# romanwerpachowski/ML

Hardware: NVIDIA B200
Metric: em_point_components_per_second (higher is better)
Workload: dtype f64

## Files before the change

### ml_b200/csrc/em.cu

```cuda
#include <algorithm>
#include <cmath>
#include <cstring>
#include <limits>

#include "em_direct.cuh"
#include "em_split.cuh"
#include "fastmath.cuh"
#include "internal.h"

namespace mlb {

constexpr int kTile = 64;
constexpr int kEmThreads = 128;
constexpr int kLogBatch = 16;

#ifdef MLB_EM_LIBM_EXP
#define MLB_EM_EXP(x) exp(x)
#else
#define MLB_EM_EXP(x) exp_nonpositive((x), etab)
#endif
#ifndef MLB_EM_MINB_SMALL
#define MLB_EM_MINB_SMALL 4
#endif

// ... 27 lines not shown
    int chunk;
    int n_chunks;
    unsigned* counter;
    const double* r_in;
    long long r_ld;
    double* r_out;
    long long r_out_ld;
    unsigned* labels_out;
    long long range_begin, range_count;
};

__device__ __forceinline__ long long min64(long long a, long long b) { return a < b ? a : b; }

__device__ __forceinline__ void dmma(double (&acc)[2], double a, double b)
{
    asm("mma.sync.aligned.m8n8k4.row.col.f64.f64.f64.f64 {%0,%1}, {%2}, {%3}, {%0,%1};" : "+d"(acc[0]), "+d"(acc[1]) : "d"(a), "d"(b));
}

template <int NT>
__device__ __forceinline__ void load_theta_frag(const double* thE, int j, int lane, double (&bf)[NT])
{
    if constexpr (NT == 1) {
        bf[0] = thE[j * 32 + lane];
    } else {
#pragma unroll
        for (int h = 0; h < NT / 2; ++h) {
            const double2 v = reinterpret_cast<const double2*>(thE)[(j * (NT / 2) + h) * 32 + lane];
            bf[2 * h] = v.x;
            bf[2 * h + 1] = v.y;
        }
    }
}

template <int DP, int KP, int MODE>
__global__ void __launch_bounds__(kEmThreads, (DP * KP <= 128 || MODE == 2) ? MLB_EM_MINB_SMALL : 2) em_kernel(const EmArgs p)
{
    constexpr int NT = KP / 8, DQ = DP / 4, NE = em_ne(DP), NM = em_nm(DP);
    constexpr int ZS = DP + 4, RS = KP + 4;
    constexpr int WN = (NM >= 8 || NT == 1) ? 1 : 2, WM = 4 / WN;
    constexpr int MW = (NM + WM - 1) / WM, NW = NT / WN;
    constexpr int SV = em_sv(DP, KP);
    constexpr int XR = kTile * DP / kEmThreads;

    extern __shared__ __align__(16) double sm[];
    double* thE = sm;
    double* cE = thE + NE * NT * 32;
    double* Zb = cE + KP;
    double* R = Zb + 2 * kTile * ZS;
    double* wl = R + kTile * RS;
    double* sh = wl + 8;
    double* etab = sh + DP;
    __shared__ int s_next;

    const int tid = threadIdx.x, lane = tid & 31, warp = tid >> 5, g = lane >> 2, c = lane & 3;
    const int d = p.d;

    if (MODE != 1)
        for (int i = tid; i < em_theta_len(DP, KP); i += kEmThreads) sm[i] = p.theta[i];
    for (int i = tid; i < 2 * kTile * ZS; i += kEmThreads) Zb[i] = 0.0;
    for (int i = tid; i < kTile * RS; i += kEmThreads) R[i] = 0.0;
    if (tid < DP) sh[tid] = tid < d ? p.shift[tid] : 0.0;
    load_exp_table(etab);

    const int wm = warp / WN, wn = warp % WN;
    int ia[MW], ib[MW];
    double sacc[MW][NW][2];
    if (MODE != 2) {
#pragma unroll
        for (int i = 0; i < MW; ++i) {
            const int mt = wm * MW + i;
            const int2 f = mt < NM ? p.feat_m[mt * 8 + g] : make_int2(DP + 1, DP + 1);
            ia[i] = f.x;
            ib[i] = f.y;
// ... 32 lines not shown
        if (tid == 0) s_next = static_cast<int>(atomicAdd(p.counter, 1u));
        __syncthreads();
        const int chunk = s_next;
        if (chunk >= p.n_chunks) break;
        const long long p_begin = work_begin + static_cast<long long>(chunk) * p.chunk;
        const long long p_end = min64(p_begin + p.chunk, work_end);
        const int ntiles = static_cast<int>((p_end - p_begin + kTile - 1) / kTile);

        if (MODE != 2) {
#pragma unroll
            for (int i = 0; i < MW; ++i)
#pragma unroll
                for (int nt = 0; nt < NW; ++nt) sacc[i][nt][0] = sacc[i][nt][1] = 0.0;
        }
        double ll_acc = 0.0, ll_prod = 1.0;

        load_tile(p_begin, static_cast<int>(min64(kTile, p_end - p_begin)));
        store_tile(Zb, static_cast<int>(min64(kTile, p_end - p_begin)));
        __syncthreads();

        for (int t = 0; t < ntiles; ++t) {
            double* Z = Zb + (t & 1) * kTile * ZS;
            const long long tile0 = p_begin + static_cast<long long>(t) * kTile;
            const int nvalid = static_cast<int>(min64(kTile, p_end - tile0));
            const int nvalid_next = t + 1 < ntiles ? static_cast<int>(min64(kTile, p_end - tile0 - kTile)) : 0;
            if (t + 1 < ntiles) load_tile(tile0 + kTile, nvalid_next);

            if (MODE == 1) {
                for (int idx = tid; idx < kTile * p.k; idx += kEmThreads) {
                    const int pt = idx % kTile, kk = idx / kTile;
                    R[pt * RS + kk] = pt < nvalid ? p.r_in[tile0 + pt + kk * p.r_ld] : 0.0;
                }
            } else {
                const double* z0 = Z + (warp * 16 + g) * ZS;
                const double* z1 = z0 + 8 * ZS;
                double acc[2][NT][2];
#pragma unroll
                for (int nt = 0; nt < NT; ++nt) {
                    const double2 cc = *reinterpret_cast<const double2*>(cE + 8 * nt + 2 * c);
                    acc[0][nt][0] = acc[1][nt][0] = cc.x;
                    acc[0][nt][1] = acc[1][nt][1] = cc.y;
                }
                double zc0[DQ], zc1[DQ];
#pragma unroll
                for (int m = 0; m < DQ; ++m) {
                    zc0[m] = z0[4 * m + c];
                    zc1[m] = z1[4 * m + c];
                }
                auto estep = [&](int j, double a0, double a1) {
                    double bf[NT];
                    load_theta_frag<NT>(thE, j, lane, bf);
#pragma unroll
                    for (int nt = 0; nt < NT; ++nt) {
                        dmma(acc[0][nt], a0, bf[nt]);
                        dmma(acc[1][nt], a1, bf[nt]);
                    }
                };
#pragma unroll
                for (int a = 0; a < DP - 4; ++a) {
                    const double za0 = z0[a], za1 = z1[a];
#pragma unroll
                    for (int m = a / 4 + 1; m < DQ; ++m) estep(em_estep_offdiag(DP, a, m), za0 * zc0[m], za1 * zc1[m]);
                }
                constexpr int J0 = em_ne_offdiag(DP);
#pragma unroll
                for (int m = 0; m < DQ; ++m) estep(J0 + m, zc0[m] * zc0[m], zc1[m] * zc1[m]);
#pragma unroll
                for (int m = 0; m < DQ; ++m) {
                    const int o = 4 * m + ((c + 1) & 3);
                    estep(J0 + DQ + m, zc0[m] * z0[o], zc1[m] * z1[o]);
                }
#pragma unroll
                for (int h = 0; h < (DQ + 1) / 2; ++h) {
                    const int mx = 2 * h + (c >> 1);
                    const int o = 4 * mx + c, o2 = 4 * mx + ((c + 2) & 3);
                    const bool live = mx < DQ;
                    const double u0 = live ? z0[o] * z0[o2] : 0.0, u1 = live ? z1[o] * z1[o2] : 0.0;
                    estep(J0 + 2 * DQ + h, u0, u1);
                }
#pragma unroll
                for (int m = 0; m < DQ; ++m) estep(NE - DQ + m, zc0[m], zc1[m]);
                double mxs[2], sums[2];
#pragma unroll
                for (int mt = 0; mt < 2; ++mt) {
#ifdef MLB_EM_FMAX_SHIFT
                    double mx = -INFINITY;
#pragma unroll
                    for (int nt = 0; nt < NT; ++nt) mx = fmax(mx, fmax(acc[mt][nt][0], acc[mt][nt][1]));
                    mx = fmax(mx, __shfl_xor_sync(0xffffffffu, mx, 1));
                    mx = fmax(mx, __shfl_xor_sync(0xffffffffu, mx, 2));
#else
                    int mkey = lse_key(acc[mt][0][0]);
#pragma unroll
                    for (int nt = 0; nt < NT; ++nt) mkey = max(mkey, max(lse_key(acc[mt][nt][0]), lse_key(acc[mt][nt][1])));
                    mkey = max(mkey, __shfl_xor_sync(0xffffffffu, mkey, 1));
                    mkey = max(mkey, __shfl_xor_sync(0xffffffffu, mkey, 2));
                    const double mx = lse_shift_of_key(mkey);
#endif
                    double sum = 0.0;
#pragma unroll
                    for (int nt = 0; nt < NT; ++nt) {
                        acc[mt][nt][0] = MLB_EM_EXP(acc[mt][nt][0] - mx);
                        acc[mt][nt][1] = MLB_EM_EXP(acc[mt][nt][1] - mx);
                        sum += acc[mt][nt][0] + acc[mt][nt][1];
                    }
                    sum += __shfl_xor_sync(0xffffffffu, sum, 1);
                    sum += __shfl_xor_sync(0xffffffffu, sum, 2);
                    mxs[mt] = mx;
                    sums[mt] = sum;
                }
                const double inv_mine = reciprocal_of_sum((c & 1) ? sums[1] : sums[0]);
                const double invs[2] = {__shfl_sync(0xffffffffu, inv_mine, lane & ~1), __shfl_sync(0xffffffffu, inv_mine, lane | 1)};
#pragma unroll
                for (int mt = 0; mt < 2; ++mt) {
                    const int pl = warp * 16 + mt * 8 + g;
                    const double inv = invs[mt];
                    if (c == 0 && pl < nvalid) {
                        ll_acc += mxs[mt];
                        ll_prod *= sums[mt];
                    }
                    if (MODE == 0) {
#pragma unroll
                        for (int nt = 0; nt < NT; ++nt)
                            *reinterpret_cast<double2*>(R + pl * RS + 8 * nt + 2 * c) = make_double2(acc[mt][nt][0] * inv, acc[mt][nt][1] * inv);
                    } else {
                        double best = -1.0;
                        unsigned best_k = 0xffffffffu;
#pragma unroll
                        for (int nt = 0; nt < NT; ++nt)
#pragma unroll
                            for (int e = 0; e < 2; ++e) {
                                const int kk = 8 * nt + 2 * c + e;
                                const double r = acc[mt][nt][e] * inv;
                                if (kk < p.k) {
                                    if (pl < nvalid && p.r_out) p.r_out[(tile0 - p.range_begin) + pl + kk * p.r_out_ld] = r;
                                    if (r > best) { best = r; best_k = kk; }
                                }
                            }
#pragma unroll
                        for (int off = 1; off <= 2; off <<= 1) {
                            const double ob = __shfl_xor_sync(0xffffffffu, best, off);
                            const unsigned ok = __shfl_xor_sync(0xffffffffu, best_k, off);
                            if (ob > best || (ob == best && ok < best_k)) { best = ob; best_k = ok; }
// ... 16 lines not shown
                        if (wm * MW + i < NM) {
                            const double af = zp[ia[i]] * zp[ib[i]];
#pragma unroll
                            for (int nt = 0; nt < NW; ++nt) dmma(sacc[i][nt], af, bf[nt]);
                        }
                    }
                }
            }
            if (MODE != 1 && ((t & (kLogBatch - 1)) == kLogBatch - 1 || t + 1 == ntiles)) {
                ll_acc += log(ll_prod);
                ll_prod = 1.0;
            }
            if (t + 1 < ntiles) store_tile(Zb + ((t + 1) & 1) * kTile * ZS, nvalid_next);
            __syncthreads();
        }

        if (MODE != 2) {
            double* out = p.partials + static_cast<long long>(chunk) * SV;
#pragma unroll
            for (int i = 0; i < MW; ++i) {
                const int mt = wm * MW + i;
                if (mt < NM) {
#pragma unroll
                    for (int nt = 0; nt < NW; ++nt)
                        *reinterpret_cast<double2*>(out + (mt * 8 + g) * KP + (wn * NW + nt) * 8 + 2 * c) = make_double2(sacc[i][nt][0], sacc[i][nt][1]);
                }
            }
#pragma unroll
            for (int off = 16; off >= 1; off >>= 1) ll_acc += __shfl_xor_sync(0xffffffffu, ll_acc, off);
            if (lane == 0) wl[warp] = ll_acc;
            __syncthreads();
            if (tid == 0) out[NM * 8 * KP] = (wl[0] + wl[1]) + (wl[2] + wl[3]);
            if (tid >= 1 && tid < 8) out[NM * 8 * KP + tid] = 0.0;
        }
    }
}

#include "em_small.cuh"

struct EmFinalizeArgs {
    const double* vsum;
    const double* dstats;
    const double* shift;
    int d, k, DP, KP, SV;
    int DPd, dSV;
    long long n_total;
    const int2* feat_m;
    const int2* feat_e;
    int nm8, ne;
    double* means;
    double* covs;
    double* weights;
    double* inv_covs;
    double* sqrt_dets;
    double* theta_out;
    double* dimg_out;
    double* kappa_out;
    int p_in_smem;
    double* ll_ring;
    unsigned long long* ll_counter;
    int ll_ring_len;
};

__global__ void em_finalize_kernel(const EmFinalizeArgs p)
{
    extern __shared__ double fs[];
// ... 161 lines not shown
    if (p.ll_ring && (p.vsum || p.dstats) && kc == 0 && tid == 0) {
        const double ll_sum = p.vsum ? tree8(p.vsum + (p.SV - 8), p.SV) : tree8(p.dstats + (p.dSV - 8), p.dSV);
        const unsigned long long idx = *p.ll_counter;
        p.ll_ring[idx % p.ll_ring_len] = ll_sum / static_cast<double>(p.n_total) - 0.5 * d * log(2.0 * 3.14159265358979323846);
        *p.ll_counter = idx + 1;
    }
}

__global__ void selftest_exp_kernel(const double* x, long long n, double* out)
{
    __shared__ double etab[kExpTableSize];
    load_exp_table(etab);
    __syncthreads();
    const long long i = static_cast<long long>(blockIdx.x) * blockDim.x + threadIdx.x;
    if (i < n) out[i] = exp_nonpositive(x[i], etab);
}


using EmKernelFn = void (*)(EmArgs);

template <int MODE>
static EmKernelFn em_kernel_for(int DP, int KP)
{
#define MLB_EM_CASE(D_, K_) if (DP == D_ && KP == K_) return em_kernel<D_, K_, MODE>;
#define MLB_EM_SMALL_CASE(D_, K_) if (DP == D_ && KP == K_) return em_small_kernel<D_, K_, MODE>;
    MLB_EM_SMALL_CASE(4, 8) MLB_EM_SMALL_CASE(4, 16) MLB_EM_SMALL_CASE(4, 32)
    MLB_EM_SMALL_CASE(8, 8) MLB_EM_SMALL_CASE(8, 16) MLB_EM_SMALL_CASE(8, 32)
    MLB_EM_CASE(16, 8) MLB_EM_CASE(16, 16) MLB_EM_CASE(16, 32)
#undef MLB_EM_CASE
#undef MLB_EM_SMALL_CASE
    return nullptr;
}

struct EmGpu {
    double* theta[2] = {nullptr, nullptr};
    double* params = nullptr;
    double* partials = nullptr;
    double* vsum = nullptr;
    double* ll = nullptr;
    unsigned long long* ll_counter = nullptr;
    int2* feat_m = nullptr;
    int2* feat_e = nullptr;
    unsigned* counter = nullptr;
    double* stage = nullptr;
    unsigned* stage_labels = nullptr;
    int grid = 0;
    double* r = nullptr;
    double* ll_tile = nullptr;
    int2* feat_e_off = nullptr;
    int grid_e = 0, grid_m = 0;
    KernelTimer timer;
};

using EmSplitKernelFn = void (*)(EmSplitArgs);

struct EmDirectGpu {
    double* img = nullptr;
    double* kappa = nullptr;
    double* r = nullptr;
    double* ll_tile = nullptr;
    double* partials = nullptr;
    double* vsum = nullptr;
    long long* sc_begin = nullptr;
    int2* tile_tab = nullptr;
    int n_sc = 0;
    int grid_e = 0, grid_m = 0;
};

struct EmDirect {
    bool capable = false;
    bool ready = false;
    int DP = 0, NB = 0, KPr = 0, IMG = 0, L = 0, SVd = 0;
    int cb = 1, cg = 1, tiles_per_range = 0, n_ranges = 1;
    size_t smem_e = 0, smem_m = 0;
    int64_t sc_bounds[kVirtualShards + 1] = {};
    std::vector<EmDirectGpu> gpus;
    ReduceScratch scratch;
};

constexpr int kDirectMaxDim = 128;
constexpr double kKappaDirect = 3.0e5;

constexpr int kLlRing = 4096;
constexpr long long kStagePoints = 1 << 20;

}

using namespace mlb;

struct mlb_em {
    mlb_ctx* ctx = nullptr;
    mlb_data* data = nullptr;
    int d = 0, k = 0, DP = 0, KP = 0, NT = 0, NE = 0, NM = 0, SV = 0;
    std::vector<int2> feat_m, feat_e;
    std::vector<EmGpu> gpus;
    int cur = 0;
    bool have_params = false, have_step = false;
    int last_path = 0;
    int64_t direct_steps = 0;
    int64_t launches = 0;
    int64_t steps_done = 0;
    EmKernelFn fn_step = nullptr, fn_mstep = nullptr, fn_emit = nullptr;
    int path = 1;
    EmDirect dr;
    int forced_path = 0;
    int route = 1;
    double kappa_max = 0.0;
    bool r_direct_valid = false;
    double* kappa_host = nullptr;
    EmSplitKernelFn fn_split_e = nullptr, fn_split_m = nullptr;
    size_t smem_split_e = 0, smem_split_m = 0;
    size_t smem_fused = 0;
    int MW = 4;
    cudaGraphExec_t step_graph[2] = {nullptr, nullptr};
    int64_t launches_per_step = 0;
    int plain_steps = 0;
    ReduceScratch reduce_scratch;

    double* means(int g) const { return gpus[g].params; }
    double* covs(int g) const { return gpus[g].params + d * k; }
    double* weights(int g) const { return covs(g) + static_cast<size_t>(k) * d * d; }
    double* inv_covs(int g) const { return weights(g) + k; }
    double* sqrt_dets(int g) const { return inv_covs(g) + static_cast<size_t>(k) * d * d; }
    size_t params_len() const { return static_cast<size_t>(d) * k + 2 * static_cast<size_t>(k) * d * d + 2 * k; }
};

namespace mlb {

static int pad_to(int v, const int* options, int n)
{
    for (int i = 0; i < n; ++i)
        if (v <= options[i]) return options[i];
    return 0;
}

static EmArgs base_args(const mlb_em* em, int g)
{
    const DataShard& sh = em->data->shards[g];
    const EmGpu& eg = em->gpus[g];
    EmArgs a{};
    a.x = sh.x;
    a.n_local = sh.n();
    a.d = em->d;
    a.k = em->k;
    a.shift = sh.shift;
    a.theta = eg.theta[em->cur];
    a.feat_m = eg.feat_m;
    a.partials = eg.partials;
    a.chunk = em->data->lay.chunk;
    a.n_chunks = static_cast<int>(sh.n_chunks());
    a.counter = eg.counter;
    return a;
}

static int launch_em(mlb_em* em, EmKernelFn fn, const EmArgs& a, int g, int grid)
{
    Gpu& gpu = em->ctx->gpus[g];
    MLB_CUDA(cudaMemsetAsync(a.counter, 0, sizeof(unsigned), gpu.stream));
    if (a.n_chunks > 0) {
        const bool timed = fn == em->fn_step;
        if (timed) MLB_TRY(em->gpus[g].timer.begin(gpu.stream));
        fn<<<std::min(grid, a.n_chunks), em->DP <= 8 ? kSmallThreads : kEmThreads, em->smem_fused, gpu.stream>>>(a);
        MLB_CUDA(cudaGetLastError());
        if (timed) MLB_TRY(em->gpus[g].timer.end(gpu.stream));
        ++em->launches;
    }
    return MLB_OK;
}

static EmSplitArgs split_args(const mlb_em* em, int g, const double* theta)
{
    const DataShard& sh = em->data->shards[g];
    const EmGpu& eg = em->gpus[g];
    EmSplitArgs a{};
    a.x = sh.x;
    a.n_local = sh.n();
    a.d = em->d; a.k = em->k; a.DP = em->DP; a.KP = em->KP;
    a.shift = sh.shift;
    a.theta = theta;
    a.feat_e = eg.feat_e_off;
    a.feat_m = eg.feat_m;
    a.ne = em->NE; a.nm = em->NM;
    a.r = eg.r;
    a.partials = eg.partials;
    a.ll_tile = eg.ll_tile;
    a.sv = em->SV;
    a.chunk = em->data->lay.chunk;
    a.n_chunks = static_cast<int>(sh.n_chunks());
    a.counter = eg.counter;
    return a;
}

static int launch_split(mlb_em* em, int g, const double* theta, bool run_e, bool timed)
{
    Gpu& gpu = em->ctx->gpus[g];
    EmGpu& eg = em->gpus[g];
    const EmSplitArgs a = split_args(em, g, theta);
    if (a.n_chunks == 0) return MLB_OK;
    if (timed) MLB_TRY(eg.timer.begin(gpu.stream));
    if (run_e) {
        MLB_CUDA(cudaMemsetAsync(a.counter, 0, sizeof(unsigned), gpu.stream));
        const long long e_items = static_cast<long long>(a.n_chunks) * (a.chunk / kSpTile);
        em->fn_split_e<<<static_cast<unsigned>(std::min<long long>(eg.grid_e, e_items)), kSpThreads, em->smem_split_e, gpu.stream>>>(a);
        MLB_CUDA(cudaGetLastError());
        ++em->launches;
    }
    const int ngroups = em->KP / (em->NT * 8), nslabs = (em->NM + 4 * em->MW - 1) / (4 * em->MW);
    const long long nitems = static_cast<long long>(a.n_chunks) * nslabs * ngroups;
    MLB_REQUIRE(nitems < (1ll << 31), "EM split path: too many work items");
    MLB_CUDA(cudaMemsetAsync(a.counter, 0, sizeof(unsigned), gpu.stream));
    em->fn_split_m<<<static_cast<unsigned>(std::min<long long>(eg.grid_m, nitems)), kSpThreads, em->smem_split_m, gpu.stream>>>(a);
    MLB_CUDA(cudaGetLastError());
    ++em->launches;
    if (timed) MLB_TRY(eg.timer.end(gpu.stream));
    return MLB_OK;
}

static int launch_pass(mlb_em* em, int g, const double* theta, bool timed)
{
    if (em->path == 2) return launch_split(em, g, theta, true, timed);
    EmArgs a = base_args(em, g);
    a.theta = theta;
    return launch_em(em, em->fn_step, a, g, em->gpus[g].grid);
}

static EmFinalizeArgs finalize_args(const mlb_em* em, int g, int stats, int theta_slot, bool want_ll)
{
    const EmGpu& eg = em->gpus[g];
    EmFinalizeArgs f{};
    f.vsum = stats == 1 ? eg.vsum : nullptr;
    f.shift = em->data->shards[g].shift;
    f.d = em->d; f.k = em->k; f.DP = em->DP; f.KP = em->KP; f.SV = em->SV;
    f.n_total = em->data->lay.n_total;
    f.feat_m = eg.feat_m; f.feat_e = eg.feat_e;
    f.nm8 = em->NM * 8; f.ne = em->NE;
    f.means = em->means(g); f.covs = em->covs(g); f.weights = em->weights(g);
    f.inv_covs = em->inv_covs(g); f.sqrt_dets = em->sqrt_dets(g);
    f.theta_out = em->path ? eg.theta[theta_slot] : nullptr;
    if (em->dr.capable) {
        const EmDirectGpu& dg = em->dr.gpus[g];
        f.DPd = em->dr.DP; f.dSV = em->dr.SVd;
        f.dstats = stats == 2 ? dg.vsum : nullptr;
        f.dimg_out = dg.img;
        f.kappa_out = dg.kappa;
    }
    f.ll_ring = want_ll ? eg.ll : nullptr;
    f.ll_counter = eg.ll_counter;
    f.ll_ring_len = kLlRing;
    return f;
}

static size_t finalize_smem(const mlb_em* em, bool* p_in_smem)
{
    const size_t d = static_cast<size_t>(em->d);
    const size_t with_p = sizeof(double) * (2 * d * d + 3 * d), without = sizeof(double) * (d * d + 3 * d);
    const bool fits = with_p <= 200 * 1024;
// ... 407 lines not shown
    MLB_CUDA(cudaMemcpy(out, dy, sizeof(double) * n, cudaMemcpyDeviceToHost));
    MLB_CUDA(cudaFree(dx));
    MLB_CUDA(cudaFree(dy));
    return MLB_OK;
}

int mlb_em_create(mlb_ctx* ctx, mlb_data* data, int k, mlb_em** out)
{
    MLB_ENTER(ctx);
    MLB_REQUIRE(ctx && data && out, "mlb_em_create: null argument");
    MLB_REQUIRE(data->ctx == ctx, "mlb_em_create: data belongs to another context");
    MLB_REQUIRE(k >= 1, "mlb_em_create: number of components must be positive");
    MLB_REQUIRE(data->d <= kDirectMaxDim, "mlb_em_create: D=%d not supported by this build (D <= %d)", data->d, kDirectMaxDim);
    static const int dps[] = {4, 8, 16}, kps[] = {8, 16, 32};
    const bool fused = data->d <= 16 && k <= 32;
    const bool split = !fused && data->d <= 64 && k <= 256;
    int DP = 0, KP = 0, NT = 0;
    if (fused) {
        DP = pad_to(data->d, dps, 3);
        KP = pad_to(k, kps, 3);
        NT = KP / 8;
    } else if (split) {
        DP = (data->d + 3) / 4 * 4;
        const int KG = k > 32 ? 64 : (k > 16 ? 32 : 16);
        KP = (k + KG - 1) / KG * KG;
        NT = KG / 8;
    }
    auto* em = new mlb_em;
    em->ctx = ctx; em->data = data; em->d = data->d; em->k = k;
    em->path = fused ? 1 : split ? 2 : 0;
    em->route = em->path ? em->path : 3;
    if (const char* env = std::getenv("MLB200_EM_PATH"))
        if (std::strcmp(env, "direct") == 0) em->forced_path = 3;
    if (em->path) {
        em->DP = DP; em->KP = KP; em->NT = NT; em->NE = em_ne(DP); em->NM = em_nm(DP); em->SV = em_sv(DP, KP);
    }
    if (fused) {
        em->fn_step = em_kernel_for<0>(DP, KP);
        em->fn_mstep = em_kernel_for<1>(DP, KP);
        em->fn_emit = em_kernel_for<2>(DP, KP);
        em->smem_fused = DP <= 8 ? em_small_smem_bytes(DP, KP) : em_smem_bytes(DP, KP);
    } else if (split) {
        em->fn_split_e = NT == 8 ? em_split_e_kernel<8> : NT == 4 ? em_split_e_kernel<4> : em_split_e_kernel<2>;
        int best_waste = 1 << 30;
        for (int mw = 3; mw <= 5; ++mw) {
            const int slabs = (em->NM + 4 * mw - 1) / (4 * mw), waste = slabs * 4 * mw - em->NM;
            if (waste <= best_waste) { best_waste = waste; em->MW = mw; }
        }
        if (NT == 8) em->fn_split_m = em->MW == 3 ? em_split_m_kernel<8, 3> : em->MW == 4 ? em_split_m_kernel<8, 4> : em_split_m_kernel<8, 5>;
        else if (NT == 4) em->fn_split_m = em->MW == 3 ? em_split_m_kernel<4, 3> : em->MW == 4 ? em_split_m_kernel<4, 4> : em_split_m_kernel<4, 5>;
        else em->fn_split_m = em->MW == 3 ? em_split_m_kernel<2, 3> : em->MW == 4 ? em_split_m_kernel<2, 4> : em_split_m_kernel<2, 5>;
        em->smem_split_e = em_split_e_smem(NT, DP, KP);
        em->smem_split_m = em_split_m_smem(NT, DP);
    }
    if (em->path) {
        em->feat_e.assign(static_cast<size_t>(em->NE) * 4, make_int2(-1, -1));
        const int DQ = DP / 4, J0 = em_ne_offdiag(DP);
        auto put = [&](int j, int c, int a, int b) { em->feat_e[static_cast<size_t>(j) * 4 + c] = make_int2(std::min(a, b), std::max(a, b)); };
        for (int a = 0; a < DP - 4; ++a)
            for (int m = a / 4 + 1; m < DQ; ++m)
                for (int c = 0; c < 4; ++c) put(em_estep_offdiag(DP, a, m), c, a, 4 * m + c);
        for (int m = 0; m < DQ; ++m)
            for (int c = 0; c < 4; ++c) {
                put(J0 + m, c, 4 * m + c, 4 * m + c);
                put(J0 + DQ + m, c, 4 * m + c, 4 * m + ((c + 1) & 3));
            }
        for (int h = 0; h < (DQ + 1) / 2; ++h)
            for (int c = 0; c < 4; ++c) {
                const int mx = 2 * h + (c >> 1);
                if (mx < DQ) put(J0 + 2 * DQ + h, c, 4 * mx + c, 4 * mx + ((c + 2) & 3));
            }
// ... 48 lines not shown
    int rc = for_each_gpu(ctx, [&](int g, Gpu& gpu) -> int {
        EmGpu& eg = em->gpus[g];
        EmDirectGpu& dg = em->dr.gpus[g];
        const DataShard& sh = data->shards[g];
        MLB_CUDA(cudaMallocFromPoolAsync(&eg.params, sizeof(double) * em->params_len(), gpu.pool, gpu.stream));
        MLB_CUDA(cudaMallocFromPoolAsync(&eg.ll, sizeof(double) * kLlRing, gpu.pool, gpu.stream));
        MLB_CUDA(cudaMallocFromPoolAsync(&eg.ll_counter, sizeof(unsigned long long), gpu.pool, gpu.stream));
        MLB_CUDA(cudaMemsetAsync(eg.ll_counter, 0, sizeof(unsigned long long), gpu.stream));
        MLB_CUDA(cudaMallocFromPoolAsync(&eg.counter, sizeof(unsigned), gpu.pool, gpu.stream));
        MLB_CUDA(cudaMallocFromPoolAsync(&dg.img, sizeof(double) * static_cast<size_t>(k) * em->dr.IMG, gpu.pool, gpu.stream));
        MLB_CUDA(cudaMallocFromPoolAsync(&dg.kappa, sizeof(double) * k, gpu.pool, gpu.stream));
        MLB_CUDA(cudaMemsetAsync(dg.kappa, 0, sizeof(double) * k, gpu.stream));
        {
            const size_t fin_smem = finalize_smem(em, nullptr);
            if (fin_smem > 48 * 1024)
                MLB_CUDA(cudaFuncSetAttribute(reinterpret_cast<const void*>(em_finalize_kernel), cudaFuncAttributeMaxDynamicSharedMemorySize, static_cast<int>(fin_smem)));
        }
        int sms = 0;
        MLB_CUDA(cudaDeviceGetAttribute(&sms, cudaDevAttrMultiProcessorCount, gpu.device));
        if (em->path) {
            const size_t theta_len = static_cast<size_t>(em_theta_len(DP, KP));
            MLB_CUDA(cudaMallocFromPoolAsync(&eg.theta[0], sizeof(double) * theta_len, gpu.pool, gpu.stream));
            MLB_CUDA(cudaMallocFromPoolAsync(&eg.theta[1], sizeof(double) * theta_len, gpu.pool, gpu.stream));
            MLB_CUDA(cudaMallocFromPoolAsync(&eg.partials, sizeof(double) * std::max<int64_t>(1, sh.n_chunks()) * em->SV, gpu.pool, gpu.stream));
            MLB_CUDA(cudaMallocFromPoolAsync(&eg.vsum, sizeof(double) * kVirtualShards * em->SV, gpu.pool, gpu.stream));
            MLB_CUDA(cudaMallocFromPoolAsync(&eg.feat_m, sizeof(int2) * em->feat_m.size(), gpu.pool, gpu.stream));
            MLB_CUDA(cudaMallocFromPoolAsync(&eg.feat_e, sizeof(int2) * em->feat_e.size(), gpu.pool, gpu.stream));
            MLB_CUDA(cudaMemsetAsync(eg.vsum, 0, sizeof(double) * kVirtualShards * em->SV, gpu.stream));
            MLB_CUDA(cudaMemcpyAsync(eg.feat_m, em->feat_m.data(), sizeof(int2) * em->feat_m.size(), cudaMemcpyHostToDevice, gpu.stream));
            MLB_CUDA(cudaMemcpyAsync(eg.feat_e, em->feat_e.data(), sizeof(int2) * em->feat_e.size(), cudaMemcpyHostToDevice, gpu.stream));
        }
        if (em->path == 1) {
            const size_t smem = em->smem_fused;
            for (EmKernelFn fn : {em->fn_step, em->fn_mstep, em->fn_emit})
                MLB_CUDA(cudaFuncSetAttribute(reinterpret_cast<const void*>(fn), cudaFuncAttributeMaxDynamicSharedMemorySize, static_cast<int>(smem)));
            int per_sm = 0;
            MLB_CUDA(cudaOccupancyMaxActiveBlocksPerMultiprocessor(&per_sm, reinterpret_cast<const void*>(em->fn_step), em->DP <= 8 ? kSmallThreads : kEmThreads, smem));
            MLB_REQUIRE(per_sm >= 1, "mlb_em_create: EM kernel does not fit on an SM");
            eg.grid = per_sm * sms;
        } else if (em->path == 2) {
            std::vector<int2> off(em->feat_e.size());
            for (size_t i = 0; i < off.size(); ++i) off[i] = em->feat_e[i].x < 0 ? make_int2(DP + 1, DP + 1) : em->feat_e[i];
            MLB_CUDA(cudaMallocFromPoolAsync(&eg.feat_e_off, sizeof(int2) * off.size(), gpu.pool, gpu.stream));
            MLB_CUDA(cudaMemcpyAsync(eg.feat_e_off, off.data(), sizeof(int2) * off.size(), cudaMemcpyHostToDevice, gpu.stream));
            MLB_CUDA(cudaStreamSynchronize(gpu.stream));
            MLB_CUDA(cudaMallocFromPoolAsync(&eg.r, sizeof(double) * std::max<int64_t>(1, sh.n()) * KP, gpu.pool, gpu.stream));
            {
                const size_t n_tiles = static_cast<size_t>(std::max<int64_t>(1, sh.n_chunks())) * (data->lay.chunk / kSpTile);
                MLB_CUDA(cudaMallocFromPoolAsync(&eg.ll_tile, sizeof(double) * n_tiles, gpu.pool, gpu.stream));
                MLB_CUDA(cudaMemsetAsync(eg.ll_tile, 0, sizeof(double) * n_tiles, gpu.stream));
            }
            MLB_CUDA(cudaMemsetAsync(eg.partials, 0, sizeof(double) * std::max<int64_t>(1, sh.n_chunks()) * em->SV, gpu.stream));
            MLB_CUDA(cudaFuncSetAttribute(reinterpret_cast<const void*>(em->fn_split_e), cudaFuncAttributeMaxDynamicSharedMemorySize, static_cast<int>(em->smem_split_e)));
            MLB_CUDA(cudaFuncSetAttribute(reinterpret_cast<const void*>(em->fn_split_m), cudaFuncAttributeMaxDynamicSharedMemorySize, static_cast<int>(em->smem_split_m)));
            int per_e = 0, per_m = 0;
            MLB_CUDA(cudaOccupancyMaxActiveBlocksPerMultiprocessor(&per_e, reinterpret_cast<const void*>(em->fn_split_e), kSpThreads, em->smem_split_e));
            MLB_CUDA(cudaOccupancyMaxActiveBlocksPerMultiprocessor(&per_m, reinterpret_cast<const void*>(em->fn_split_m), kSpThreads, em->smem_split_m));
            MLB_REQUIRE(per_e >= 1 && per_m >= 1, "mlb_em_create: EM kernels do not fit on an SM (D=%d, K=%d)", em->d, em->k);
            eg.grid_e = per_e * sms;
            eg.grid_m = per_m * sms;
        }
        MLB_CUDA(cudaStreamSynchronize(gpu.stream));
        return MLB_OK;
    });
    if (rc != MLB_OK) { mlb_em_destroy(em); return rc; }
    *out = em;
    return MLB_OK;
}

int mlb_em_destroy(mlb_em* em)
{
    MLB_ENTER(em ? em->ctx : nullptr);
// ... 110 lines not shown
    if (covariances) MLB_CUDA(cudaMemcpyAsync(covariances, em->covs(0), sizeof(double) * em->k * em->d * em->d, cudaMemcpyDeviceToHost, gpu.stream));
    if (weights) MLB_CUDA(cudaMemcpyAsync(weights, em->weights(0), sizeof(double) * em->k, cudaMemcpyDeviceToHost, gpu.stream));
    MLB_CUDA(cudaStreamSynchronize(gpu.stream));
    return MLB_OK;
}

int mlb_em_get_precisions(mlb_em* em, double* inverse_covariances, double* sqrt_determinants)
{
    MLB_ENTER(em ? em->ctx : nullptr);
    MLB_REQUIRE(em, "mlb_em_get_precisions: null argument");
    if (!em->have_params) { set_error("mlb_em_get_precisions: parameters not set"); return MLB_ESTATE; }
    Gpu& gpu = em->ctx->gpus[0];
    MLB_CUDA(cudaSetDevice(gpu.device));
    if (inverse_covariances)
        MLB_CUDA(cudaMemcpyAsync(inverse_covariances, em->inv_covs(0), sizeof(double) * em->k * em->d * em->d, cudaMemcpyDeviceToHost, gpu.stream));
    if (sqrt_determinants) MLB_CUDA(cudaMemcpyAsync(sqrt_determinants, em->sqrt_dets(0), sizeof(double) * em->k, cudaMemcpyDeviceToHost, gpu.stream));
    MLB_CUDA(cudaStreamSynchronize(gpu.stream));
    return MLB_OK;
}

int mlb_em_sample_covariance(mlb_em* em, double* cov_out)
{
    MLB_ENTER(em ? em->ctx : nullptr);
    MLB_REQUIRE(em && cov_out, "mlb_em_sample_covariance: null argument");
    if (em->path == 0 || em->forced_path == 3) return direct_sample_covariance(em, cov_out);
    const int d = em->d, DP = em->DP;
    const bool narrow = em->path == 1 && em->KP > 8;
    const int KP = narrow ? 8 : em->KP, SV = narrow ? em_sv(DP, 8) : em->SV;
    std::vector<double> theta(em_theta_len(DP, KP), 0.0);
    for (int kk = 1; kk < KP; ++kk) theta[static_cast<size_t>(em->NE) * (KP / 8) * 32 + kk] = -std::numeric_limits<double>::infinity();
    MLB_TRY(for_each_gpu(em->ctx, [&](int g, Gpu& gpu) -> int {
        MLB_CUDA(cudaMemcpyAsync(em->gpus[g].theta[em->cur ^ 1], theta.data(), sizeof(double) * theta.size(), cudaMemcpyHostToDevice, gpu.stream));
        if (!narrow) return launch_pass(em, g, em->gpus[g].theta[em->cur ^ 1], false);
        const EmKernelFn fn = em_kernel_for<0>(DP, 8);
        const size_t smem = DP <= 8 ? em_small_smem_bytes(DP, 8) : em_smem_bytes(DP, 8);
        MLB_CUDA(cudaFuncSetAttribute(reinterpret_cast<const void*>(fn), cudaFuncAttributeMaxDynamicSharedMemorySize, static_cast<int>(smem)));
        int per_sm = 0, sms = 0;
        MLB_CUDA(cudaOccupancyMaxActiveBlocksPerMultiprocessor(&per_sm, reinterpret_cast<const void*>(fn), em->DP <= 8 ? kSmallThreads : kEmThreads, smem));
        MLB_CUDA(cudaDeviceGetAttribute(&sms, cudaDevAttrMultiProcessorCount, gpu.device));
        MLB_REQUIRE(per_sm >= 1, "mlb_em_sample_covariance: kernel does not fit on an SM");
        EmArgs a = base_args(em, g);
        a.theta = em->gpus[g].theta[em->cur ^ 1];
        a.k = 1;
        MLB_CUDA(cudaMemsetAsync(a.counter, 0, sizeof(unsigned), gpu.stream));
        if (a.n_chunks > 0) {
            fn<<<std::min(per_sm * sms, a.n_chunks), em->DP <= 8 ? kSmallThreads : kEmThreads, smem, gpu.stream>>>(a);
            MLB_CUDA(cudaGetLastError());
            ++em->launches;
        }
        return MLB_OK;
    }));
    if (em->path == 2) em->have_step = false;
    std::vector<double*> partials, vsum;
    for (EmGpu& eg : em->gpus) { partials.push_back(eg.partials); vsum.push_back(eg.vsum); }
    MLB_TRY(reduce_and_exchange(em->data, partials, vsum, SV, em->reduce_scratch));
    em->launches += static_cast<int64_t>(em->ctx->gpus.size());
    std::vector<double> host(static_cast<size_t>(kVirtualShards) * SV);
    Gpu& gpu0 = em->ctx->gpus[0];
    MLB_CUDA(cudaSetDevice(gpu0.device));
    MLB_CUDA(cudaMemcpyAsync(host.data(), em->gpus[0].vsum, sizeof(double) * host.size(), cudaMemcpyDeviceToHost, gpu0.stream));
    MLB_TRY(mlb_ctx_synchronize(em->ctx));
    double count = 0;
    std::vector<double> m1(d, 0.0), m2(static_cast<size_t>(d) * d, 0.0);
    for (size_t f = 0; f < em->feat_m.size(); ++f) {
        const int2 ab = em->feat_m[f];
        const double val = tree8(host.data() + f * KP, SV);
        if (ab.x == DP && ab.y == DP) count = val;
        else if (ab.y == DP && ab.x < d) m1[ab.x] = val;
        else if (ab.x < d && ab.y < d) { m2[ab.x + static_cast<size_t>(ab.y) * d] = val; m2[ab.y + static_cast<size_t>(ab.x) * d] = val; }
    }
    for (int a = 0; a < d; ++a)
        for (int b = 0; b < d; ++b)
            cov_out[a + static_cast<size_t>(b) * d] = (m2[a + static_cast<size_t>(b) * d] - m1[a] * m1[b] / count) / (count - 1.0);
    return MLB_OK;
}

int mlb_em_mstep_from_responsibilities(mlb_em* em, const double* resp, int64_t ld)
{
    MLB_ENTER(em ? em->ctx : nullptr);
// ... 281 lines not shown
```

Measured before the change: 48.59.

## Add warp-specialized EM kernel with producer E-step and consumer M-step warps

```diff
diff --git a/ml_b200/csrc/em.cu b/ml_b200/csrc/em.cu
--- a/ml_b200/csrc/em.cu
+++ b/ml_b200/csrc/em.cu
@@ -83,13 +83,97 @@
     }
 }
 
+__host__ __device__ constexpr int em_wn(int DP, int KP) { return (em_nm(DP) >= 8 || KP == 8) ? 1 : 2; }
+__host__ __device__ constexpr int em_mw(int DP, int KP) { return (em_nm(DP) + 4 / em_wn(DP, KP) - 1) / (4 / em_wn(DP, KP)); }
+
+template <int DP, int KP>
+__device__ __forceinline__ void em_estep_warp(const double* z0, const double* thE, const double* cE, const double* etab, int lane,
+                                              double (&acc)[2][KP / 8][2], double (&mxs)[2], double (&sums)[2])
+{
+    constexpr int NT = KP / 8, DQ = DP / 4, NE = em_ne(DP), ZS = DP + 4;
+    const int c = lane & 3;
+    const double* z1 = z0 + 8 * ZS;
+#pragma unroll
+    for (int nt = 0; nt < NT; ++nt) {
+        const double2 cc = *reinterpret_cast<const double2*>(cE + 8 * nt + 2 * c);
+        acc[0][nt][0] = acc[1][nt][0] = cc.x;
+        acc[0][nt][1] = acc[1][nt][1] = cc.y;
+    }
+    double zc0[DQ], zc1[DQ];
+#pragma unroll
+    for (int m = 0; m < DQ; ++m) {
+        zc0[m] = z0[4 * m + c];
+        zc1[m] = z1[4 * m + c];
+    }
+    auto estep = [&](int j, double a0, double a1) {
+        double bf[NT];
+        load_theta_frag<NT>(thE, j, lane, bf);
+#pragma unroll
+        for (int nt = 0; nt < NT; ++nt) {
+            dmma(acc[0][nt], a0, bf[nt]);
+            dmma(acc[1][nt], a1, bf[nt]);
+        }
+    };
+#pragma unroll
+    for (int a = 0; a < DP - 4; ++a) {
+        const double za0 = z0[a], za1 = z1[a];
+#pragma unroll
+        for (int m = a / 4 + 1; m < DQ; ++m) estep(em_estep_offdiag(DP, a, m), za0 * zc0[m], za1 * zc1[m]);
+    }
+    constexpr int J0 = em_ne_offdiag(DP);
+#pragma unroll
+    for (int m = 0; m < DQ; ++m) estep(J0 + m, zc0[m] * zc0[m], zc1[m] * zc1[m]);
+#pragma unroll
+    for (int m = 0; m < DQ; ++m) {
+        const int o = 4 * m + ((c + 1) & 3);
+        estep(J0 + DQ + m, zc0[m] * z0[o], zc1[m] * z1[o]);
+    }
+#pragma unroll
+    for (int h = 0; h < (DQ + 1) / 2; ++h) {
+        const int mx = 2 * h + (c >> 1);
+        const int o = 4 * mx + c, o2 = 4 * mx + ((c + 2) & 3);
+        const bool live = mx < DQ;
+        const double u0 = live ? z0[o] * z0[o2] : 0.0, u1 = live ? z1[o] * z1[o2] : 0.0;
+        estep(J0 + 2 * DQ + h, u0, u1);
+    }
+#pragma unroll
+    for (int m = 0; m < DQ; ++m) estep(NE - DQ + m, zc0[m], zc1[m]);
+#pragma unroll
+    for (int mt = 0; mt < 2; ++mt) {
+#ifdef MLB_EM_FMAX_SHIFT
+        double mx = -INFINITY;
+#pragma unroll
+        for (int nt = 0; nt < NT; ++nt) mx = fmax(mx, fmax(acc[mt][nt][0], acc[mt][nt][1]));
+        mx = fmax(mx, __shfl_xor_sync(0xffffffffu, mx, 1));
+        mx = fmax(mx, __shfl_xor_sync(0xffffffffu, mx, 2));
+#else
+        int mkey = lse_key(acc[mt][0][0]);
+#pragma unroll
+        for (int nt = 0; nt < NT; ++nt) mkey = max(mkey, max(lse_key(acc[mt][nt][0]), lse_key(acc[mt][nt][1])));
+        mkey = max(mkey, __shfl_xor_sync(0xffffffffu, mkey, 1));
+        mkey = max(mkey, __shfl_xor_sync(0xffffffffu, mkey, 2));
+        const double mx = lse_shift_of_key(mkey);
+#endif
+        double sum = 0.0;
+#pragma unroll
+        for (int nt = 0; nt < NT; ++nt) {
+            acc[mt][nt][0] = MLB_EM_EXP(acc[mt][nt][0] - mx);
+            acc[mt][nt][1] = MLB_EM_EXP(acc[mt][nt][1] - mx);
+            sum += acc[mt][nt][0] + acc[mt][nt][1];
+        }
+        sum += __shfl_xor_sync(0xffffffffu, sum, 1);
+        sum += __shfl_xor_sync(0xffffffffu, sum, 2);
+        mxs[mt] = mx;
+        sums[mt] = sum;
+    }
+}
+
 template <int DP, int KP, int MODE>
 __global__ void __launch_bounds__(kEmThreads, (DP * KP <= 128 || MODE == 2) ? MLB_EM_MINB_SMALL : 2) em_kernel(const EmArgs p)
 {
-    constexpr int NT = KP / 8, DQ = DP / 4, NE = em_ne(DP), NM = em_nm(DP);
+    constexpr int NT = KP / 8, NE = em_ne(DP), NM = em_nm(DP);
     constexpr int ZS = DP + 4, RS = KP + 4;
-    constexpr int WN = (NM >= 8 || NT == 1) ? 1 : 2, WM = 4 / WN;
-    constexpr int MW = (NM + WM - 1) / WM, NW = NT / WN;
+    constexpr int WN = em_wn(DP, KP), MW = em_mw(DP, KP), NW = NT / WN;
     constexpr int SV = em_sv(DP, KP);
     constexpr int XR = kTile * DP / kEmThreads;
 
@@ -188,83 +272,8 @@
                     R[pt * RS + kk] = pt < nvalid ? p.r_in[tile0 + pt + kk * p.r_ld] : 0.0;
                 }
             } else {
-                const double* z0 = Z + (warp * 16 + g) * ZS;
-                const double* z1 = z0 + 8 * ZS;
-                double acc[2][NT][2];
-#pragma unroll
-                for (int nt = 0; nt < NT; ++nt) {
-                    const double2 cc = *reinterpret_cast<const double2*>(cE + 8 * nt + 2 * c);
-                    acc[0][nt][0] = acc[1][nt][0] = cc.x;
-                    acc[0][nt][1] = acc[1][nt][1] = cc.y;
-                }
-                double zc0[DQ], zc1[DQ];
-#pragma unroll
-                for (int m = 0; m < DQ; ++m) {
-                    zc0[m] = z0[4 * m + c];
-                    zc1[m] = z1[4 * m + c];
-                }
-                auto estep = [&](int j, double a0, double a1) {
-                    double bf[NT];
-                    load_theta_frag<NT>(thE, j, lane, bf);
-#pragma unroll
-                    for (int nt = 0; nt < NT; ++nt) {
-                        dmma(acc[0][nt], a0, bf[nt]);
-                        dmma(acc[1][nt], a1, bf[nt]);
-                    }
-                };
-#pragma unroll
-                for (int a = 0; a < DP - 4; ++a) {
-                    const double za0 = z0[a], za1 = z1[a];
-#pragma unroll
-                    for (int m = a / 4 + 1; m < DQ; ++m) estep(em_estep_offdiag(DP, a, m), za0 * zc0[m], za1 * zc1[m]);
-                }
-                constexpr int J0 = em_ne_offdiag(DP);
-#pragma unroll
-                for (int m = 0; m < DQ; ++m) estep(J0 + m, zc0[m] * zc0[m], zc1[m] * zc1[m]);
-#pragma unroll
-                for (int m = 0; m < DQ; ++m) {
-                    const int o = 4 * m + ((c + 1) & 3);
-                    estep(J0 + DQ + m, zc0[m] * z0[o], zc1[m] * z1[o]);
-                }
-#pragma unroll
-                for (int h = 0; h < (DQ + 1) / 2; ++h) {
-                    const int mx = 2 * h + (c >> 1);
-                    const int o = 4 * mx + c, o2 = 4 * mx + ((c + 2) & 3);
-                    const bool live = mx < DQ;
-                    const double u0 = live ? z0[o] * z0[o2] : 0.0, u1 = live ? z1[o] * z1[o2] : 0.0;
-                    estep(J0 + 2 * DQ + h, u0, u1);
-                }
-#pragma unroll
-                for (int m = 0; m < DQ; ++m) estep(NE - DQ + m, zc0[m], zc1[m]);
-                double mxs[2], sums[2];
-#pragma unroll
-                for (int mt = 0; mt < 2; ++mt) {
-#ifdef MLB_EM_FMAX_SHIFT
-                    double mx = -INFINITY;
-#pragma unroll
-                    for (int nt = 0; nt < NT; ++nt) mx = fmax(mx, fmax(acc[mt][nt][0], acc[mt][nt][1]));
-                    mx = fmax(mx, __shfl_xor_sync(0xffffffffu, mx, 1));
-                    mx = fmax(mx, __shfl_xor_sync(0xffffffffu, mx, 2));
-#else
-                    int mkey = lse_key(acc[mt][0][0]);
-#pragma unroll
-                    for (int nt = 0; nt < NT; ++nt) mkey = max(mkey, max(lse_key(acc[mt][nt][0]), lse_key(acc[mt][nt][1])));
-                    mkey = max(mkey, __shfl_xor_sync(0xffffffffu, mkey, 1));
-                    mkey = max(mkey, __shfl_xor_sync(0xffffffffu, mkey, 2));
-                    const double mx = lse_shift_of_key(mkey);
-#endif
-                    double sum = 0.0;
-#pragma unroll
-                    for (int nt = 0; nt < NT; ++nt) {
-                        acc[mt][nt][0] = MLB_EM_EXP(acc[mt][nt][0] - mx);
-                        acc[mt][nt][1] = MLB_EM_EXP(acc[mt][nt][1] - mx);
-                        sum += acc[mt][nt][0] + acc[mt][nt][1];
-                    }
-                    sum += __shfl_xor_sync(0xffffffffu, sum, 1);
-                    sum += __shfl_xor_sync(0xffffffffu, sum, 2);
-                    mxs[mt] = mx;
-                    sums[mt] = sum;
-                }
+                double acc[2][NT][2], mxs[2], sums[2];
+                em_estep_warp<DP, KP>(Z + (warp * 16 + g) * ZS, thE, cE, etab, lane, acc, mxs, sums);
                 const double inv_mine = reciprocal_of_sum((c & 1) ? sums[1] : sums[0]);
                 const double invs[2] = {__shfl_sync(0xffffffffu, inv_mine, lane & ~1), __shfl_sync(0xffffffffu, inv_mine, lane | 1)};
 #pragma unroll
@@ -347,6 +356,202 @@
             __syncthreads();
             if (tid == 0) out[NM * 8 * KP] = (wl[0] + wl[1]) + (wl[2] + wl[3]);
             if (tid >= 1 && tid < 8) out[NM * 8 * KP + tid] = 0.0;
+        }
+    }
+}
+
+constexpr int kWsThreads = 256;
+constexpr int kWsSlots = 2;
+
+constexpr size_t em_ws_smem_bytes(int DP, int KP)
+{
+    return sizeof(double) * (em_theta_len(DP, KP) + kWsSlots * kTile * ((DP + 4) + (KP + 4)) + 8 + DP + kExpTableSize);
+}
+
+__device__ __forceinline__ void named_bar_sync(int id, int nthreads) { asm volatile("bar.sync %0, %1;" ::"r"(id), "r"(nthreads) : "memory"); }
+__device__ __forceinline__ void named_bar_arrive(int id, int nthreads) { asm volatile("bar.arrive %0, %1;" ::"r"(id), "r"(nthreads) : "memory"); }
+
+template <int DP, int KP>
+__global__ void __launch_bounds__(kWsThreads, 2) em_ws_kernel(const EmArgs p)
+{
+    constexpr int NT = KP / 8, NM = em_nm(DP);
+    constexpr int ZS = DP + 4, RS = KP + 4;
+    constexpr int WN = em_wn(DP, KP), MW = em_mw(DP, KP), NW = NT / WN;
+    constexpr int SV = em_sv(DP, KP);
+    constexpr int XR = 16 * DP / 32;
+    constexpr int kFull = 1, kEmpty = 1 + kWsSlots, kEGroup = 1 + 2 * kWsSlots;
+
+    extern __shared__ __align__(16) double sm[];
+    double* thE = sm;
+    double* cE = thE + em_ne(DP) * NT * 32;
+    double* Zr = cE + KP;
+    double* Rr = Zr + kWsSlots * kTile * ZS;
+    double* wl = Rr + kWsSlots * kTile * RS;
+    double* sh = wl + 8;
+    double* etab = sh + DP;
+    __shared__ int s_next;
+    __shared__ int s_meta[kWsSlots][2];
+
+    const int tid = threadIdx.x, lane = tid & 31, warp = tid >> 5, g = lane >> 2, c = lane & 3;
+    const int d = p.d;
+
+    for (int i = tid; i < em_theta_len(DP, KP); i += kWsThreads) sm[i] = p.theta[i];
+    for (int i = tid; i < kWsSlots * kTile * (ZS + RS); i += kWsThreads) Zr[i] = 0.0;
+    if (tid < DP) sh[tid] = tid < d ? p.shift[tid] : 0.0;
+    load_exp_table(etab);
+    __syncthreads();
+
+    if (warp < 4) {
+        double xr[XR];
+        auto load_tile = [&](long long point0, int nvalid) {
+            const double* xg = p.x + (point0 + 16 * warp) * d;
+            const int nel = (nvalid - 16 * warp) * d;
+#pragma unroll
+            for (int r = 0; r < XR; ++r) {
+                const int e = lane + 32 * r;
+                xr[r] = e < nel ? xg[e] : 0.0;
+            }
+        };
+        auto store_tile = [&](double* Z, int nvalid) {
+            const int nel = nvalid * d;
+#pragma unroll
+            for (int r = 0; r < XR; ++r) {
+                const int el = lane + 32 * r;
+                if (el < 16 * d) {
+                    const int e = 16 * warp * d + el;
+                    const int pt = (d == DP) ? e / DP : FastDiv(d).div(e);
+                    const int dm = e - pt * d;
+                    Z[pt * ZS + dm] = e < nel ? xr[r] - sh[dm] : 0.0;
+                }
+            }
+            if (lane < 16) Z[(16 * warp + lane) * ZS + DP] = 16 * warp + lane < nvalid ? 1.0 : 0.0;
+        };
+
+        int q = 0;
+        for (int chunk = -1;;) {
+            named_bar_sync(kEGroup, 128);
+            if (tid == 0) {
+                if (chunk >= 0) {
+                    double* out = p.partials + static_cast<long long>(chunk) * SV + NM * 8 * KP;
+                    out[0] = (wl[0] + wl[1]) + (wl[2] + wl[3]);
+#pragma unroll
+                    for (int i = 1; i < 8; ++i) out[i] = 0.0;
+                }
+                s_next = static_cast<int>(atomicAdd(p.counter, 1u));
+            }
+            named_bar_sync(kEGroup, 128);
+            chunk = s_next;
+            if (chunk >= p.n_chunks) break;
+            const long long p_begin = static_cast<long long>(chunk) * p.chunk;
+            const long long p_end = min64(p_begin + p.chunk, p.n_local);
+            const int ntiles = static_cast<int>((p_end - p_begin + kTile - 1) / kTile);
+            double ll_acc = 0.0, ll_prod = 1.0;
+
+            load_tile(p_begin, static_cast<int>(min64(kTile, p_end - p_begin)));
+            for (int t = 0; t < ntiles; ++t, ++q) {
+                const int slot = q % kWsSlots;
+                double* Z = Zr + slot * kTile * ZS;
+                double* R = Rr + slot * kTile * RS;
+                const long long tile0 = p_begin + static_cast<long long>(t) * kTile;
+                const int nvalid = static_cast<int>(min64(kTile, p_end - tile0));
+
+                named_bar_sync(kEmpty + slot, kWsThreads);
+                store_tile(Z, nvalid);
+                if (tid == 0) {
+                    s_meta[slot][0] = chunk;
+                    s_meta[slot][1] = t + 1 == ntiles;
+                }
+                if (t + 1 < ntiles) load_tile(tile0 + kTile, static_cast<int>(min64(kTile, p_end - tile0 - kTile)));
+                __syncwarp();
+
+                double acc[2][NT][2], mxs[2], sums[2];
+                em_estep_warp<DP, KP>(Z + (warp * 16 + g) * ZS, thE, cE, etab, lane, acc, mxs, sums);
+                const double inv_mine = reciprocal_of_sum((c & 1) ? sums[1] : sums[0]);
+                const double invs[2] = {__shfl_sync(0xffffffffu, inv_mine, lane & ~1), __shfl_sync(0xffffffffu, inv_mine, lane | 1)};
+#pragma unroll
+                for (int mt = 0; mt < 2; ++mt) {
+                    const int pl = warp * 16 + mt * 8 + g;
+                    const double inv = invs[mt];
+                    if (c == 0 && pl < nvalid) {
+                        ll_acc += mxs[mt];
+                        ll_prod *= sums[mt];
+                    }
+#pragma unroll
+                    for (int nt = 0; nt < NT; ++nt)
+                        *reinterpret_cast<double2*>(R + pl * RS + 8 * nt + 2 * c) = make_double2(acc[mt][nt][0] * inv, acc[mt][nt][1] * inv);
+                }
+                if ((t & (kLogBatch - 1)) == kLogBatch - 1 || t + 1 == ntiles) {
+                    ll_acc += log(ll_prod);
+                    ll_prod = 1.0;
+                }
+                named_bar_arrive(kFull + slot, kWsThreads);
+            }
+#pragma unroll
+            for (int off = 16; off >= 1; off >>= 1) ll_acc += __shfl_xor_sync(0xffffffffu, ll_acc, off);
+            if (lane == 0) wl[warp] = ll_acc;
+        }
+        const int slot = q % kWsSlots;
+        named_bar_sync(kEmpty + slot, kWsThreads);
+        if (tid == 0) s_meta[slot][0] = -1;
+        named_bar_arrive(kFull + slot, kWsThreads);
+        for (int s = 1; s <= kWsSlots; ++s) named_bar_sync(kEmpty + (slot + s) % kWsSlots, kWsThreads);
+    } else {
+        const int wm = (warp - 4) / WN, wn = (warp - 4) % WN;
+        int ia[MW], ib[MW];
+#pragma unroll
+        for (int i = 0; i < MW; ++i) {
+            const int mt = wm * MW + i;
+            const int2 f = mt < NM ? p.feat_m[mt * 8 + g] : make_int2(DP + 1, DP + 1);
+            ia[i] = f.x;
+            ib[i] = f.y;
+        }
+        double sacc[MW][NW][2];
+#pragma unroll
+        for (int i = 0; i < MW; ++i)
+#pragma unroll
+            for (int nt = 0; nt < NW; ++nt) sacc[i][nt][0] = sacc[i][nt][1] = 0.0;
+
+        for (int s = 0; s < kWsSlots; ++s) named_bar_arrive(kEmpty + s, kWsThreads);
+        for (int q = 0;; ++q) {
+            const int slot = q % kWsSlots;
+            named_bar_sync(kFull + slot, kWsThreads);
+            const int chunk = s_meta[slot][0], last = s_meta[slot][1];
+            if (chunk >= 0) {
+                const double* Z = Zr + slot * kTile * ZS;
+                const double* R = Rr + slot * kTile * RS;
+#pragma unroll 4
+                for (int s = 0; s < kTile / 4; ++s) {
+                    const double* zp = Z + (4 * s + c) * ZS;
+                    const double* rp = R + (4 * s + c) * RS + wn * NW * 8 + g;
+                    double bf[NW];
+#pragma unroll
+                    for (int nt = 0; nt < NW; ++nt) bf[nt] = rp[8 * nt];
+#pragma unroll
+                    for (int i = 0; i < MW; ++i) {
+                        if (wm * MW + i < NM) {
+                            const double af = zp[ia[i]] * zp[ib[i]];
+#pragma unroll
+                            for (int nt = 0; nt < NW; ++nt) dmma(sacc[i][nt], af, bf[nt]);
+                        }
+                    }
+                }
+            }
+            named_bar_arrive(kEmpty + slot, kWsThreads);
+            if (chunk < 0) break;
+            if (last) {
+                double* out = p.partials + static_cast<long long>(chunk) * SV;
+#pragma unroll
+                for (int i = 0; i < MW; ++i) {
+                    const int mt = wm * MW + i;
+                    if (mt < NM) {
+#pragma unroll
+                        for (int nt = 0; nt < NW; ++nt) {
+                            *reinterpret_cast<double2*>(out + (mt * 8 + g) * KP + (wn * NW + nt) * 8 + 2 * c) = make_double2(sacc[i][nt][0], sacc[i][nt][1]);
+                            sacc[i][nt][0] = sacc[i][nt][1] = 0.0;
+                        }
+                    }
+                }
+            }
         }
     }
 }
@@ -574,6 +779,21 @@
     return nullptr;
 }
 
+struct EmStepKernel {
+    EmKernelFn fn;
+    int threads;
+    size_t smem;
+};
+
+static EmStepKernel em_step_kernel_for(int DP, int KP, bool lockstep)
+{
+    if (DP == 16 && !lockstep) {
+        if (KP == 16) return {em_ws_kernel<16, 16>, kWsThreads, em_ws_smem_bytes(16, 16)};
+        if (KP == 32) return {em_ws_kernel<16, 32>, kWsThreads, em_ws_smem_bytes(16, 32)};
+    }
+    return {em_kernel_for<0>(DP, KP), DP <= 8 ? kSmallThreads : kEmThreads, DP <= 8 ? em_small_smem_bytes(DP, KP) : em_smem_bytes(DP, KP)};
+}
+
 struct EmGpu {
     double* theta[2] = {nullptr, nullptr};
     double* params = nullptr;
@@ -587,6 +807,7 @@
     double* stage = nullptr;
     unsigned* stage_labels = nullptr;
     int grid = 0;
+    int grid_step = 0;
     double* r = nullptr;
     double* ll_tile = nullptr;
     int2* feat_e_off = nullptr;
@@ -653,6 +874,9 @@
     EmSplitKernelFn fn_split_e = nullptr, fn_split_m = nullptr;
     size_t smem_split_e = 0, smem_split_m = 0;
     size_t smem_fused = 0;
+    bool lockstep = false;
+    int step_threads = 0;
+    size_t smem_step = 0;
     int MW = 4;
     cudaGraphExec_t step_graph[2] = {nullptr, nullptr};
     int64_t launches_per_step = 0;
@@ -702,7 +926,8 @@
     if (a.n_chunks > 0) {
         const bool timed = fn == em->fn_step;
         if (timed) MLB_TRY(em->gpus[g].timer.begin(gpu.stream));
-        fn<<<std::min(grid, a.n_chunks), em->DP <= 8 ? kSmallThreads : kEmThreads, em->smem_fused, gpu.stream>>>(a);
+        const int threads = timed ? em->step_threads : em->DP <= 8 ? kSmallThreads : kEmThreads;
+        fn<<<std::min(grid, a.n_chunks), threads, timed ? em->smem_step : em->smem_fused, gpu.stream>>>(a);
         MLB_CUDA(cudaGetLastError());
         if (timed) MLB_TRY(em->gpus[g].timer.end(gpu.stream));
         ++em->launches;
@@ -763,7 +988,7 @@
     if (em->path == 2) return launch_split(em, g, theta, true, timed);
     EmArgs a = base_args(em, g);
     a.theta = theta;
-    return launch_em(em, em->fn_step, a, g, em->gpus[g].grid);
+    return launch_em(em, em->fn_step, a, g, em->gpus[g].grid_step);
 }
 
 static EmFinalizeArgs finalize_args(const mlb_em* em, int g, int stats, int theta_slot, bool want_ll)
@@ -1237,11 +1462,16 @@
     em->route = em->path ? em->path : 3;
     if (const char* env = std::getenv("MLB200_EM_PATH"))
         if (std::strcmp(env, "direct") == 0) em->forced_path = 3;
+    if (const char* env = std::getenv("MLB200_EM_FUSED"))
+        em->lockstep = std::strcmp(env, "lockstep") == 0;
     if (em->path) {
         em->DP = DP; em->KP = KP; em->NT = NT; em->NE = em_ne(DP); em->NM = em_nm(DP); em->SV = em_sv(DP, KP);
     }
     if (fused) {
-        em->fn_step = em_kernel_for<0>(DP, KP);
+        const EmStepKernel sk = em_step_kernel_for(DP, KP, em->lockstep);
+        em->fn_step = sk.fn;
+        em->step_threads = sk.threads;
+        em->smem_step = sk.smem;
         em->fn_mstep = em_kernel_for<1>(DP, KP);
         em->fn_emit = em_kernel_for<2>(DP, KP);
         em->smem_fused = DP <= 8 ? em_small_smem_bytes(DP, KP) : em_smem_bytes(DP, KP);
@@ -1356,12 +1586,17 @@
         }
         if (em->path == 1) {
             const size_t smem = em->smem_fused;
-            for (EmKernelFn fn : {em->fn_step, em->fn_mstep, em->fn_emit})
+            for (EmKernelFn fn : {em->fn_mstep, em->fn_emit})
                 MLB_CUDA(cudaFuncSetAttribute(reinterpret_cast<const void*>(fn), cudaFuncAttributeMaxDynamicSharedMemorySize, static_cast<int>(smem)));
-            int per_sm = 0;
-            MLB_CUDA(cudaOccupancyMaxActiveBlocksPerMultiprocessor(&per_sm, reinterpret_cast<const void*>(em->fn_step), em->DP <= 8 ? kSmallThreads : kEmThreads, smem));
-            MLB_REQUIRE(per_sm >= 1, "mlb_em_create: EM kernel does not fit on an SM");
+            MLB_CUDA(cudaFuncSetAttribute(reinterpret_cast<const void*>(em->fn_step), cudaFuncAttributeMaxDynamicSharedMemorySize, static_cast<int>(em->smem_step)));
+            const EmKernelFn lockstep_fn = em_kernel_for<0>(DP, KP);
+            MLB_CUDA(cudaFuncSetAttribute(reinterpret_cast<const void*>(lockstep_fn), cudaFuncAttributeMaxDynamicSharedMemorySize, static_cast<int>(smem)));
+            int per_sm = 0, per_sm_step = 0;
+            MLB_CUDA(cudaOccupancyMaxActiveBlocksPerMultiprocessor(&per_sm, reinterpret_cast<const void*>(lockstep_fn), em->DP <= 8 ? kSmallThreads : kEmThreads, smem));
+            MLB_CUDA(cudaOccupancyMaxActiveBlocksPerMultiprocessor(&per_sm_step, reinterpret_cast<const void*>(em->fn_step), em->step_threads, em->smem_step));
+            MLB_REQUIRE(per_sm >= 1 && per_sm_step >= 1, "mlb_em_create: EM kernel does not fit on an SM");
             eg.grid = per_sm * sms;
+            eg.grid_step = per_sm_step * sms;
         } else if (em->path == 2) {
             std::vector<int2> off(em->feat_e.size());
             for (size_t i = 0; i < off.size(); ++i) off[i] = em->feat_e[i].x < 0 ? make_int2(DP + 1, DP + 1) : em->feat_e[i];
@@ -1538,11 +1773,12 @@
     MLB_TRY(for_each_gpu(em->ctx, [&](int g, Gpu& gpu) -> int {
         MLB_CUDA(cudaMemcpyAsync(em->gpus[g].theta[em->cur ^ 1], theta.data(), sizeof(double) * theta.size(), cudaMemcpyHostToDevice, gpu.stream));
         if (!narrow) return launch_pass(em, g, em->gpus[g].theta[em->cur ^ 1], false);
-        const EmKernelFn fn = em_kernel_for<0>(DP, 8);
-        const size_t smem = DP <= 8 ? em_small_smem_bytes(DP, 8) : em_smem_bytes(DP, 8);
+        const EmStepKernel sk = em_step_kernel_for(DP, 8, em->lockstep);
+        const EmKernelFn fn = sk.fn;
+        const size_t smem = sk.smem;
         MLB_CUDA(cudaFuncSetAttribute(reinterpret_cast<const void*>(fn), cudaFuncAttributeMaxDynamicSharedMemorySize, static_cast<int>(smem)));
         int per_sm = 0, sms = 0;
-        MLB_CUDA(cudaOccupancyMaxActiveBlocksPerMultiprocessor(&per_sm, reinterpret_cast<const void*>(fn), em->DP <= 8 ? kSmallThreads : kEmThreads, smem));
+        MLB_CUDA(cudaOccupancyMaxActiveBlocksPerMultiprocessor(&per_sm, reinterpret_cast<const void*>(fn), sk.threads, smem));
         MLB_CUDA(cudaDeviceGetAttribute(&sms, cudaDevAttrMultiProcessorCount, gpu.device));
         MLB_REQUIRE(per_sm >= 1, "mlb_em_sample_covariance: kernel does not fit on an SM");
         EmArgs a = base_args(em, g);
@@ -1550,7 +1786,7 @@
         a.k = 1;
         MLB_CUDA(cudaMemsetAsync(a.counter, 0, sizeof(unsigned), gpu.stream));
         if (a.n_chunks > 0) {
-            fn<<<std::min(per_sm * sms, a.n_chunks), em->DP <= 8 ? kSmallThreads : kEmThreads, smem, gpu.stream>>>(a);
+            fn<<<std::min(per_sm * sms, a.n_chunks), sk.threads, smem, gpu.stream>>>(a);
             MLB_CUDA(cudaGetLastError());
             ++em->launches;
         }
```

Result: faster. 49.88 (median of 6 runs) (+2.6%).
